# ktzsh/object-tracking

Measured on AMD Instinct MI355X. Metric: frames/sec detect+track @416x416, higher is better.
Workload: dtype f32; 1 GPU; BASELINE.json configs[2]: MultiObjDetTracker (YOLOv2 C=12 + ConvLSTM2D(512) + 1x1 + decode/NMS + track ids), 48 clips x 30 frames per GPU per step, 416x416 uint8; the synthetic head is calibrated to 32 CANDIDATE boxes per frame, of which about 20 survive NMS (config.boxes_per_frame: measured).  The step computes the model's TRACKING output, the one MultiObjDetTracker.predict reads (MultiObjDetTrac; parallelism=clip-shard x1

## Files before the change

object_tracking_amd/build.py:

```python
import os
import subprocess
import sys
from concurrent.futures import ThreadPoolExecutor

HERE = os.path.dirname(os.path.abspath(__file__))
CSRC = os.path.join(HERE, "csrc")
LIB = os.path.join(HERE, "libmi355_dt.so")
HIPCC = os.environ.get("HIPCC", "/opt/rocm/bin/hipcc")

SOURCES = {
    "conv_igemm.hip": [],
    "conv1.hip": [],
    "winograd.hip": [],
    "wino4s_fused.hip": ["-fno-slp-vectorize"],
    "wino_gemm_s3.hip": [],
    "conv3_h2.hip": [],
    "ingest.hip": [],
    "extract.hip": [],
    "exchange.hip": [],
    "decode.hip": ["-ffp-contract=off"],
    "associate.hip": ["-ffp-contract=off"],
    "score.hip": ["-ffp-contract=off"],
    "identity.hip": ["-ffp-contract=off"],
    "detscore.hip": ["-ffp-contract=off"],
    "targets.hip": ["-ffp-contract=off"],
    "recurrent.hip": [],
    "stream_state.hip": [],
    "network.hip": [],
}
COMMON = ["--offload-arch=gfx950", "-O3", "-std=c++17", "-fPIC", "-fvisibility=hidden",
          "-fgpu-rdc" if False else "-fno-gpu-rdc", "-Wall", "-Wno-unused-function"]
HEADERS = [os.path.join(CSRC, "dt_internal.h"), os.path.join(HERE, "..", "include", "mi355_dt.h")]


def _stale(out, deps):
    if not os.path.exists(out):
        return True
    t = os.path.getmtime(out)
    return any(os.path.getmtime(d) > t for d in deps)


def build(force=False, verbose=False):
    objs, jobs = [], []
    for src, extra in SOURCES.items():
        s = os.path.join(CSRC, src)
        o = os.path.join(CSRC, src.replace(".hip", ".o"))
        objs.append(o)
        if force or _stale(o, [s] + HEADERS + [os.path.abspath(__file__)]):
            jobs.append([HIPCC] + COMMON + extra + ["-c", s, "-o", o])

    def run(cmd):
        if verbose:
            print(" ".join(cmd), flush=True)
        r = subprocess.run(cmd, capture_output=True, text=True)
        if r.returncode != 0:
            raise RuntimeError("hipcc failed: %s\n%s\n%s" % (" ".join(cmd), r.stdout, r.stderr))
        if verbose and r.stderr.strip():
            print(r.stderr)

    with ThreadPoolExecutor(max_workers=min(8, max(1, len(jobs)))) as ex:
        list(ex.map(run, jobs))
    if jobs or force or _stale(LIB, objs):
        run([HIPCC, "--offload-arch=gfx950", "-shared", "-fPIC", "-o", LIB] + objs)
    return LIB

# ... 4 lines not shown
```

object_tracking_amd/csrc/conv3_h2.hip:

```cpp
#include "dt_internal.h"
#include <type_traits>

typedef _Float16 c3_h8 __attribute__((ext_vector_type(8)));
typedef _Float16 c3_h4 __attribute__((ext_vector_type(4)));
typedef float c3_f16 __attribute__((ext_vector_type(16)));
typedef float c3_f4 __attribute__((ext_vector_type(4)));
typedef unsigned c3_u4 __attribute__((ext_vector_type(4)));
typedef unsigned c3_u2 __attribute__((ext_vector_type(2)));
typedef __attribute__((address_space(3))) void c3_lptr_t;
typedef const __attribute__((address_space(1))) void c3_gptr_t;

constexpr int C3_PW = 18;
#define C3_THREADS 256
#define C3_NS 3

template <int N>
__device__ __forceinline__ void c3_wait_vm() { __builtin_amdgcn_s_waitcnt(0x0f70 | (N & 15) | ((N >> 4) << 14)); }

__device__ __forceinline__ void c3_mfma(c3_f16 &c, const c3_u4 &w, const c3_u4 &a)
{
    c = __builtin_amdgcn_mfma_f32_32x32x16_f16(__builtin_bit_cast(c3_h8, a), __builtin_bit_cast(c3_h8, w), c, 0, 0, 0);
}

template <int WN, bool POOL, bool FUSE = false>
__global__ __launch_bounds__(C3_THREADS) __attribute__((amdgpu_waves_per_eu(2, 2))) void conv3_h2_kernel(Conv3H2Args p)
{
    static_assert(!FUSE || (WN == 2 && !POOL), "the fused 1x1 follows the 128-channel, un-pooled instance");
    constexpr int WM = 4 / WN;
    constexpr int TH = 4 * WM, TW = 16;
    constexpr int BN = 64 * WN;
    constexpr int PH = TH + 2, PW = C3_PW, NPIX = PH * PW;
    constexpr int PLANE = NPIX * 32;
    constexpr int PATCH = 4 * PLANE;
    constexpr int BPL = BN * 32;
    constexpr int BSTAGE = 4 * BPL;
    constexpr int PB = (4 * BN / 32) / 4;
    constexpr int NJ = (PH * 18 * 8 + C3_THREADS - 1) / C3_THREADS;
    extern __shared__ __attribute__((aligned(16))) unsigned char c3_lds[];
    unsigned char *patch = c3_lds, *bring = c3_lds + PATCH;
    float *btab = reinterpret_cast<float *>(c3_lds + PATCH + C3_NS * BSTAGE);
    [[maybe_unused]] float *btab1 = btab + BN;
    constexpr int SPL = 128 * 32;
    constexpr int BPL1 = 64 * 32;
    const int tid = threadIdx.x, lane = tid & 63, wave = tid >> 6;
    const int wm = wave % WM, wn = wave / WM;
    const int rl = lane & 31, gl = lane >> 5;

    const unsigned am = dt_amax_read(p.amax);
    const float fwd = dt_h2_base(am);
    const float inv = p.pscale[0] * dt_h2_base_inv(am);
    const int nchunk = p.Cin >> 5;
    const int ntn = (p.N + BN - 1) / BN;
    const int tiles = p.tiles_x * p.tiles_y;
    const long long items = (long long)p.B * tiles * ntn;
    const long long wterm = (long long)(9 * p.Cin / 16) * p.Np * 16;
    float out_am = 0.0f;

    long long item = blockIdx.x;
    if (item >= items) return;

    struct Unit { int b, ty0, tx0, n0, chunk; };
    auto unit_of = [&](long long it, int chunk) {
        Unit u;
        u.n0 = (int)(it % ntn) * BN;
        const long long r = it / ntn;
        const int t = (int)(r % tiles);
        u.b = (int)(r / tiles);
        u.ty0 = (t / p.tiles_x) * TH;
        u.tx0 = (t % p.tiles_x) * TW;
        u.chunk = chunk;
        return u;
    };
    c3_f4 pf[NJ];
    auto patch_request = [&](const Unit &u) {
#pragma unroll
        for (int j = 0; j < NJ; ++j) {
// ... 31 lines not shown
    int wdst[PB];
#pragma unroll
    for (int q = 0; q < PB; ++q) {
        const int pc = wave * PB + q;
        const int grp = pc % (BN / 32), ht = pc / (BN / 32);
        const int half = ht >> 1, term = ht & 1;
        wsrc[q] = p.w + term * wterm + ((long long)half * p.Np + 32 * grp + lrow) * 16 + dgran * 8;
        wdst[q] = ht * BPL + grp * 1024;
    }
    const long long wstage = (long long)2 * p.Np * 16;
    auto stage_off = [&](int n0, int chunk, int tap) { return (long long)(chunk * 9 + tap) * wstage + (long long)n0 * 16; };
    auto piece_issue = [&](int buf, long long off, int q) {
        __builtin_amdgcn_global_load_lds((c3_gptr_t *)(wsrc[q] + off), (c3_lptr_t *)(bring + buf * BSTAGE + wdst[q]), 16, 0, 0);
    };
    auto stage_issue = [&](int buf, int n0, int chunk, int tap) {
        const long long off = stage_off(n0, chunk, tap);
#pragma unroll
        for (int q = 0; q < PB; ++q) piece_issue(buf, off, q);
    };
    int offB[2];
#pragma unroll
    for (int j = 0; j < 2; ++j) {
        const int row = wn * 64 + 32 * j + rl;
        offB[j] = (2 * row + (gl ^ ((row >> 3) & 1))) * 16;
    }
    int pixA[2];
#pragma unroll
    for (int i = 0; i < 2; ++i) pixA[i] = (4 * wm + 2 * i + (rl >> 4)) * PW + (rl & 15);
    auto offA_of = [&](int i, int tap) {
        const int pix = pixA[i] + (tap / 3) * PW + tap % 3;
        return pix * 32 + ((gl ^ ((pix >> 3) & 1)) * 16);
    };

    [[maybe_unused]] const unsigned short *w1src[2] = {nullptr, nullptr};
    [[maybe_unused]] int w1dst[2] = {0, 0};
    if constexpr (FUSE) {
        const long long w1term = (long long)8 * p.Np1 * 16;
#pragma unroll
        for (int q = 0; q < 2; ++q) {
            const int pc = wave * 2 + q, grp = pc & 1, ht = pc >> 1, half = ht >> 1, term = ht & 1;
            w1src[q] = p.w1 + term * w1term + ((long long)half * p.Np1 + 32 * grp + lrow) * 16 + dgran * 8;
            w1dst[q] = ht * BPL1 + grp * 1024;
        }
        for (int i = tid; i < 64; i += C3_THREADS) btab1[i] = i < p.N1 ? p.bias1[i] : 0.0f;
    }
    auto fstage_issue = [&](int buf, int q, int k) {
        if constexpr (FUSE)
            __builtin_amdgcn_global_load_lds((c3_gptr_t *)(w1src[k] + (long long)(2 * q) * p.Np1 * 16), (c3_lptr_t *)(bring + buf * BSTAGE + w1dst[k]), 16, 0, 0);
    };
    int sbase = 0;
    auto bufof = [&](int k) { return FUSE ? (sbase + k) % C3_NS : k % C3_NS; };

    Unit cur = unit_of(item, 0);
    patch_request(cur);
    stage_issue(0, cur.n0, 0, 0);
    stage_issue(1, cur.n0, 0, 1);
    for (int i = tid; i < BN; i += C3_THREADS) btab[i] = (cur.n0 + i < p.N) ? p.bias[cur.n0 + i] : 0.0f;
    patch_store();

    c3_f16 acc[2][2];
    c3_u4 fa[2][2][2], fb[2][2][2];
    for (;;) {
        if (cur.chunk == 0) {
#pragma unroll
            for (int j = 0; j < 2; ++j)
#pragma unroll
                for (int i = 0; i < 2; ++i)
#pragma unroll
                    for (int e = 0; e < 16; ++e) acc[j][i][e] = 0.0f;
        }
        const bool last_chunk = cur.chunk == nchunk - 1;
        const long long nitem = last_chunk ? item + gridDim.x : item;
        const bool has_next = nitem < items;
        Unit nxt = cur;
        if (has_next) nxt = unit_of(nitem, last_chunk ? 0 : cur.chunk + 1);

        auto stage = [&](auto tapc) {
            constexpr int tap = decltype(tapc)::value;
            if (tap == 1 && has_next) c3_wait_vm<NJ>();
            else c3_wait_vm<0>();
            __builtin_amdgcn_s_waitcnt(0xc07f);
            __builtin_amdgcn_s_barrier();
            const bool fnext = FUSE && last_chunk && tap >= 7;
            const bool refill = tap < 7 || (has_next && !fnext);
            const long long roff = tap < 7 ? stage_off(cur.n0, cur.chunk, tap + 2) : stage_off(nxt.n0, nxt.chunk, tap - 7);
            const unsigned char *sb = bring + bufof(tap) * BSTAGE, *sn = bring + bufof(tap + 1) * BSTAGE;
            if (tap == 0) {
#pragma unroll
                for (int i = 0; i < 2; ++i)
#pragma unroll
                    for (int t = 0; t < 2; ++t) fa[0][i][t] = *reinterpret_cast<const c3_u4 *>(patch + t * PLANE + offA_of(i, 0));
#pragma unroll
                for (int j = 0; j < 2; ++j)
#pragma unroll
                    for (int t = 0; t < 2; ++t) fb[0][j][t] = *reinterpret_cast<const c3_u4 *>(sb + t * BPL + offB[j]);
            }
            int oa[2], on[2];
#pragma unroll
            for (int i = 0; i < 2; ++i) { oa[i] = offA_of(i, tap); on[i] = offA_of(i, tap < 8 ? tap + 1 : 0); }
            __builtin_amdgcn_sched_barrier(0);
#pragma unroll
            for (int hf = 0; hf < 2; ++hf) {
                const bool rd = hf == 0 || tap < 8;
#pragma unroll
                for (int m = 0; m < 12; ++m) {
                    const int pr = m >> 2, j = (m >> 1) & 1, i = m & 1;
                    c3_mfma(acc[j][i], fb[hf][j][pr == 0 ? 1 : 0], fa[hf][i][pr == 1 ? 1 : 0]);
                    if (rd && m < 8) {
                        const int k = m & 3, blk = k >> 1, t = k & 1;
                        if (m < 4) {
                            if (hf == 0) fa[1][blk][t] = *reinterpret_cast<const c3_u4 *>(patch + (2 + t) * PLANE + oa[blk]);
                            else fa[0][blk][t] = *reinterpret_cast<const c3_u4 *>(patch + t * PLANE + on[blk]);
                        } else {
                            if (hf == 0) fb[1][blk][t] = *reinterpret_cast<const c3_u4 *>(sb + (2 + t) * BPL + offB[blk]);
                            else fb[0][blk][t] = *reinterpret_cast<const c3_u4 *>(sn + t * BPL + offB[blk]);
                        }
                    }
                    if (hf == 0 && m >= 8 && m - 8 < PB && refill) piece_issue(bufof(tap + 2), roff, m - 8);
                    if (FUSE && hf == 0 && m >= 8 && m - 8 < 2 && fnext) fstage_issue(bufof(tap + 2), tap - 7, m - 8);
                    __builtin_amdgcn_sched_barrier(0);
                }
                if (tap == 0 && hf == 0 && has_next) { patch_request(nxt); __builtin_amdgcn_sched_barrier(0); }
            }
        };
        stage(std::integral_constant<int, 0>{}); stage(std::integral_constant<int, 1>{}); stage(std::integral_constant<int, 2>{});
        stage(std::integral_constant<int, 3>{}); stage(std::integral_constant<int, 4>{}); stage(std::integral_constant<int, 5>{});
        stage(std::integral_constant<int, 6>{}); stage(std::integral_constant<int, 7>{}); stage(std::integral_constant<int, 8>{});

        if (FUSE && last_chunk) {
            float am = 0.0f;
#pragma unroll
            for (int j = 0; j < 2; ++j) {
                const float bl = btab[wn * 64 + 32 * j + rl];
#pragma unroll
                for (int i = 0; i < 2; ++i)
#pragma unroll
                    for (int e = 0; e < 16; ++e) {
                        const float z = __builtin_fmaf(acc[j][i][e], inv, bl);
                        const float y = fmaxf(z, z * p.slope);
                        acc[j][i][e] = y;
                        am = fmaxf(am, fabsf(y));
                    }
            }
#pragma unroll
            for (int o = 32; o; o >>= 1) am = fmaxf(am, __shfl_xor(am, o));
            if (lane == 0) btab1[64 + wave] = am;
            __builtin_amdgcn_s_waitcnt(0xc07f);
            __builtin_amdgcn_s_barrier();
            const float tmax = fmaxf(fmaxf(btab1[64], btab1[65]), fmaxf(btab1[66], btab1[67]));
            const unsigned tb = __float_as_uint(tmax);
            const float f1 = dt_h2_base(tb), inv1 = p.pscale1[0] * dt_h2_base_inv(tb);
            c3_f16 acc2[2];
#pragma unroll
            for (int jn = 0; jn < 2; ++jn)
#pragma unroll
                for (int e = 0; e < 16; ++e) acc2[jn][e] = 0.0f;
            const int prow = 32 * wave + rl;
            const int offS = prow * 32 + ((gl ^ ((prow >> 3) & 1)) * 16);
            int offB1[2];
#pragma unroll
            for (int jn = 0; jn < 2; ++jn) { const int n = 32 * jn + rl; offB1[jn] = (2 * n + (gl ^ ((n >> 3) & 1))) * 16; }
#pragma unroll
            for (int q = 0; q < 4; ++q) {
                if (wn == (q >> 1)) {
                    const int j = q & 1, half = rl >> 4, g = (rl >> 3) & 1;
#pragma unroll
                    for (int i = 0; i < 2; ++i)
#pragma unroll
                        for (int r = 0; r < 16; ++r) {
                            const int pp = 64 * wm + 32 * i + 8 * (r >> 2) + 4 * gl + (r & 3);
                            const float x = acc[j][i][r] * f1;
                            const _Float16 hi = (_Float16)x;
                            const _Float16 lo = (_Float16)(x - (float)hi);
                            unsigned char *dst = patch + (half * 2) * SPL + pp * 32 + ((g ^ ((pp >> 3) & 1)) * 16) + (rl & 7) * 2;
                            *reinterpret_cast<_Float16 *>(dst) = hi;
                            *reinterpret_cast<_Float16 *>(dst + SPL) = lo;
                        }
                }
                c3_wait_vm<0>();
                __builtin_amdgcn_s_waitcnt(0xc07f);
                __builtin_amdgcn_s_barrier();
                if (q < 2) { fstage_issue(bufof(11 + q), q + 2, 0); fstage_issue(bufof(11 + q), q + 2, 1); }
                else if (has_next) stage_issue(bufof(11 + q), nxt.n0, nxt.chunk, q - 2);
                const unsigned char *sq = bring + bufof(9 + q) * BSTAGE;
#pragma unroll
                for (int hf = 0; hf < 2; ++hf) {
                    c3_u4 a2[2], b2[2][2];
#pragma unroll
                    for (int t = 0; t < 2; ++t) a2[t] = *reinterpret_cast<const c3_u4 *>(patch + (hf * 2 + t) * SPL + offS);
#pragma unroll
                    for (int jn = 0; jn < 2; ++jn)
#pragma unroll
                        for (int t = 0; t < 2; ++t) b2[jn][t] = *reinterpret_cast<const c3_u4 *>(sq + (hf * 2 + t) * BPL1 + offB1[jn]);
#pragma unroll
                    for (int jn = 0; jn < 2; ++jn) c3_mfma(acc2[jn], b2[jn][1], a2[0]);
#pragma unroll
                    for (int jn = 0; jn < 2; ++jn) c3_mfma(acc2[jn], b2[jn][0], a2[1]);
#pragma unroll
                    for (int jn = 0; jn < 2; ++jn) c3_mfma(acc2[jn], b2[jn][0], a2[0]);
                }
                if (q < 3) {
                    __builtin_amdgcn_s_waitcnt(0xc07f);
                    __builtin_amdgcn_s_barrier();
                }
            }
            sbase = (sbase + 13) % C3_NS;
            const int yb = cur.ty0 + 4 * (wave >> 1) + 2 * (wave & 1);
#pragma unroll
            for (int jn = 0; jn < 2; ++jn) {
                const int n = 32 * jn + rl;
                const float b1 = btab1[n];
                const bool nok = n < p.N1;
#pragma unroll
                for (int r = 0; r < 16; ++r) {
                    const int m = 8 * (r >> 2) + 4 * gl + (r & 3);
                    const int y = yb + (m >> 4), x = cur.tx0 + (m & 15);
                    const float z = __builtin_fmaf(acc2[jn][r], inv1, b1);
                    const float v = fmaxf(z, z * p.slope1);
                    if (nok && y < p.H && x < p.W) {
                        if (p.amax_out) out_am = fmaxf(out_am, fabsf(v));
                        __builtin_nontemporal_store(v, p.out + (long long)cur.b * p.out_bs + ((long long)y * p.W + x) * p.out_ld + n);
                    }
                }
            }
        } else if (last_chunk) {
#pragma unroll
            for (int j = 0; j < 2; ++j) {
                const int nl = wn * 64 + 32 * j + rl;
                const float bl = btab[nl];
                const bool nok = cur.n0 + nl < p.N;
#pragma unroll
                for (int i = 0; i < 2; ++i) {
#pragma unroll
                    for (int e = 0; e < 16; ++e) {
                        const float z = __builtin_fmaf(acc[j][i][e], inv, bl);
                        acc[j][i][e] = fmaxf(z, z * p.slope);
                    }
                    const int yb = cur.ty0 + 4 * wm + 2 * i;
                    if (!POOL) {
#pragma unroll
                        for (int r = 0; r < 16; ++r) {
                            const int m = 8 * (r >> 2) + 4 * gl + (r & 3);
                            const int y = yb + (m >> 4), x = cur.tx0 + (m & 15);
                            if (nok && y < p.H && x < p.W) {
                                if (p.amax_out) out_am = fmaxf(out_am, fabsf(acc[j][i][r]));
                                __builtin_nontemporal_store(acc[j][i][r], p.out + (long long)cur.b * p.out_bs + ((long long)y * p.W + x) * p.out_ld + cur.n0 + nl);
                            }
                        }
                    } else {
                        const int H2 = p.H >> 1, W2 = p.W >> 1;
                        const int y2 = yb >> 1;
#pragma unroll
                        for (int q = 0; q < 4; ++q) {
                            const int r = 2 * q;
                            const float mx = fmaxf(fmaxf(acc[j][i][r], acc[j][i][r + 1]), fmaxf(acc[j][i][r + 8], acc[j][i][r + 9]));
                            const int x2 = (cur.tx0 >> 1) + 4 * (q >> 1) + 2 * gl + (q & 1);
                            if (nok && y2 < H2 && x2 < W2) {
                                if (p.amax_out) out_am = fmaxf(out_am, fabsf(mx));
                                __builtin_nontemporal_store(mx, p.out2 + (((long long)cur.b * H2 + y2) * W2 + x2) * p.out2_ld + cur.n0 + nl);
                            }
                        }
                    }
                }
            }
        }
        if (!has_next) break;
        __builtin_amdgcn_s_waitcnt(0xc07f);
        __builtin_amdgcn_s_barrier();
        patch_store();
        if (last_chunk && nxt.n0 != cur.n0)
            for (int i = tid; i < BN; i += C3_THREADS) btab[i] = (nxt.n0 + i < p.N) ? p.bias[nxt.n0 + i] : 0.0f;
        item = nitem;
        cur = nxt;
    }
    if (p.amax_out) dt_amax_publish(p.amax_out, out_am);
}

bool conv3_h2_usable(const Conv3H2Args &a)
{
    return a.Cin % 32 == 0 && a.Cin >= 32 && a.N >= 64 && a.N % 64 == 0 && a.Np % 64 == 0 && a.in_ld % 4 == 0 && (reinterpret_cast<uintptr_t>(a.in) & 15) == 0 &&
           a.w && a.pscale && a.amax && a.bias && a.zeros && (a.out != nullptr) != (a.out2 != nullptr) && (!a.out2 || !((a.H | a.W) & 1)) &&
           (!a.w1 || (a.N == 128 && a.out && a.pscale1 && a.bias1 && a.N1 > 0 && a.N1 <= 64 && a.Np1 >= 64 && a.Np1 % 32 == 0));
}
double conv3_h2_flops(const Conv3H2Args &a)
{
    const bool wide = a.N % 128 == 0;
    const int th = wide ? 8 : 16;
    const double tiles = (double)a.B * ((a.H + th - 1) / th) * ((a.W + 15) / 16);
    return 6.0 * tiles * th * 16 * (9.0 * a.Cin * a.N + (a.w1 ? (double)a.N * 64 : 0.0));
}

template <int WN, bool POOL, bool FUSE = false>
static int c3_launch(hipStream_t st, const Conv3H2Args &a, int cus)
{
    constexpr int TH = 16 / WN, BN = 64 * WN;
    const size_t lds = (size_t)4 * (TH + 2) * C3_PW * 32 + (size_t)C3_NS * 4 * BN * 32 + BN * 4 + (FUSE ? 68 * 4 : 0);
    static PerDeviceOnce attr;
    if (attr.ensure(nullptr, [&](int) {
            return hipFuncSetAttribute(reinterpret_cast<const void *>(conv3_h2_kernel<WN, POOL, FUSE>), hipFuncAttributeMaxDynamicSharedMemorySize, (int)lds) != hipSuccess;
        }))
        return 1;
    Conv3H2Args p = a;
    p.tiles_y = (a.H + TH - 1) / TH;
// ... 28 lines not shown
```

object_tracking_amd/csrc/dt_internal.h:

```cpp
#pragma once
#include <hip/hip_runtime.h>

#include <atomic>
#include <cstdint>
#include <cstdio>
#include <map>
#include <mutex>
#include <functional>
#include <string>
#include <type_traits>
#include <vector>

#include "../../include/mi355_dt.h"

struct PerDeviceOnce {
    std::atomic<unsigned long long> mask{0};
    std::mutex mu;
    template <class F> int ensure(int *dev_out, F &&setup)
    {
        int dev = -1;
        if (hipGetDevice(&dev) != hipSuccess || dev < 0 || dev > 63) return 1;
        if (dev_out) *dev_out = dev;
        if ((mask.load(std::memory_order_acquire) >> dev) & 1ull) return 0;
        std::lock_guard<std::mutex> lk(mu);
// ... 516 lines not shown
    void reset()
    {
        if (p) (void)hipFree(p);
        p = nullptr;
    }
    hipError_t alloc(size_t n)
    {
        reset();
        const hipError_t e = hipMalloc(reinterpret_cast<void **>(&p), n * sizeof(T));
        if (e != hipSuccess) p = nullptr;
        return e;
    }
    T *get() const { return p; }
    explicit operator bool() const { return p != nullptr; }
};
static_assert(!std::is_copy_constructible<DevMem<float>>::value && !std::is_copy_assignable<DevMem<float>>::value, "a device allocation has one owner");

struct WinoWeights {
    int ts = 0;
    int cin = 0, npad = 0;
    DevMem<float> u;
    DevMem<unsigned short> s3;
    DevMem<unsigned short> h2;
    DevMem<float> h2_pscale;
};

struct ConvLayer {
    int idx = 0, ks = 0, cin = 0, cout = 0, npad = 0;
    DevMem<float> wt;
    DevMem<unsigned short> wt_s3;
    DevMem<unsigned short> bias_s3;
    DevMem<unsigned short> wt_h2;
    DevMem<float> pscale_h2;
    DevMem<unsigned short> w3_h2;
    DevMem<float> pscale_w3;
    WinoWeights wino;
    WinoWeights wino_alt;
    DevMem<float> fused4s;
    DevMem<float> bias;
    DevMem<float> scale;
    bool scale_has_zero = false;
};

struct Policy {
    int wino = 1;
    int wino_tile = 0;
    int wino_mint = 0;
    double wino_ws_gb = 96.0;
    int mosaic = -1;
    int fused4 = 1;
    int trk_merge = 1;
    int pin = 0;
    int c3h2 = 1;
    int conv_cfg = -1;
    int s3_conv1 = 1;
    int s3 = 1;
    int s3_minrows = 2048;
    int s3_minrows_h2 = 64;
    int s3_h2 = 1;
    int c3fuse = 1;
    int h2_minframes = 12;
    int s3_half = 0;
    int s3_rec_minrows = 512;
    int s3_rec_minrows_h2 = 16;
    int s3_1x1_mink = 256;
    int s3_1x1_minrows = 16384;
// ... 98 lines not shown
```

object_tracking_amd/csrc/network.hip:

```cpp
#include <algorithm>
#include <cmath>
#include <cstdarg>
#include <cstdlib>
#include <cstring>
#include <thread>

#include "dt_internal.h"

static const float BN_EPS = 1e-3f;
static const float LEAKY = 0.1f;
static char g_static_err[512] = "";

static const int TRUNK[20][5] = {
    {1, 3, 3, 32, 1},      {2, 3, 32, 64, 1},     {3, 3, 64, 128, 0},    {4, 1, 128, 64, 0},
    {5, 3, 64, 128, 1},    {6, 3, 128, 256, 0},   {7, 1, 256, 128, 0},   {8, 3, 128, 256, 1},
    {9, 3, 256, 512, 0},   {10, 1, 512, 256, 0},  {11, 3, 256, 512, 0},  {12, 1, 512, 256, 0},
    {13, 3, 256, 512, 1},  {14, 3, 512, 1024, 0}, {15, 1, 1024, 512, 0}, {16, 3, 512, 1024, 0},
    {17, 1, 1024, 512, 0}, {18, 3, 512, 1024, 0}, {19, 3, 1024, 1024, 0}, {20, 3, 1024, 1024, 0}};

static inline int round_up(int v, int m) { return (v + m - 1) / m * m; }

int dt_fail(dt_ctx *ctx, int code, const char *fmt, ...)
{
    char buf[512];
    va_list ap;
    va_start(ap, fmt);
    vsnprintf(buf, sizeof(buf), fmt, ap);
    va_end(ap);
    if (ctx) ctx->err = buf;
    else snprintf(g_static_err, sizeof(g_static_err), "%s", buf);
    return code;
}

static void graphs_clear(dt_ctx *ctx)
{
    if (ctx->graphs.empty() && ctx->graph_seen.empty()) return;
    (void)hipStreamSynchronize(ctx->stream);
    for (auto &kv : ctx->graphs) (void)hipGraphExecDestroy(kv.second);
    ctx->graphs.clear();
    ctx->graph_seen.clear();
// ... 500 lines not shown
{
    ConvLayer L;
    L.idx = idx; L.ks = ks; L.cin = cin; L.cout = cout;
    L.npad = round_up(cout, 256);
    std::vector<float> packed((size_t)L.npad * ks * ks * cin);
    pack_conv_weights(hwio, ks, cin, cout, nullptr, cin, nullptr, L.npad, scale, packed.data());
    std::vector<float> bias(L.npad, 0.0f);
    for (int c = 0; c < cout; ++c) bias[c] = bias_src[c];
    int rc = upload(ctx, L.wt, packed);
    if (rc) return rc;
    if (ks == 1 && ctx->pol.s3 != 0 && ctx->pol.s3_1x1 != 0 && cin % 32 == 0 && L.npad % 128 == 0 && cout >= 64) {
        HIP_TRY(ctx, L.wt_s3.alloc(packed.size() * 3));
        if (launch_wino_s3_pack(ctx->stream, L.wt.get(), 1, L.npad, cin, L.wt_s3.get())) return dt_fail(ctx, DT_ERR_DEVICE, "split-bf16 weight pack launch failed");
        HIP_TRY(ctx, hipStreamSynchronize(ctx->stream));
        std::vector<unsigned short> bs((size_t)3 * L.npad * 16, 0);
        for (int n = 0; n < cout; ++n) {
            unsigned short t[3];
            wino_s3_split_host(bias_src[n], t);
            for (int t3 = 0; t3 < 3; ++t3) bs[((size_t)t3 * L.npad + n) * 16] = t[t3];
        }
        if ((rc = upload(ctx, L.bias_s3, bs))) return rc;
        if (!ctx->s3_ones) {
            std::vector<float> ones((size_t)256 * 16, 0.0f);
            for (int r = 0; r < 256; ++r) ones[(size_t)r * 16] = 1.0f;
            if ((rc = upload(ctx, ctx->s3_ones, ones))) return rc;
        }
    }
    if (L.wt_s3 && ctx->pol.s3_h2 != 0) {
        HIP_TRY(ctx, L.wt_h2.alloc(packed.size() * 2));
        HIP_TRY(ctx, L.pscale_h2.alloc(1));
        if (launch_wino_h2_pack(ctx->stream, L.wt.get(), 1, L.npad, cin, 0, amax_slot(ctx, AMAX_PACK), L.wt_h2.get(), L.pscale_h2.get()))
            return dt_fail(ctx, DT_ERR_DEVICE, "fp16-form weight pack launch failed");
        HIP_TRY(ctx, hipStreamSynchronize(ctx->stream));
    }
    if (ks == 3 && (cin == 32 || cin == 64) && cout % 64 == 0 && cout <= 128 && ctx->pol.s3 != 0 && ctx->pol.s3_h2 != 0 && ctx->pol.c3h2 != 0) {
        HIP_TRY(ctx, L.w3_h2.alloc(packed.size() * 2));
        HIP_TRY(ctx, L.pscale_w3.alloc(1));
        if (launch_wino_h2_pack(ctx->stream, L.wt.get(), 1, L.npad, 9 * cin, 0, amax_slot(ctx, AMAX_PACK), L.w3_h2.get(), L.pscale_w3.get()))
            return dt_fail(ctx, DT_ERR_DEVICE, "fp16-form weight pack launch failed");
        HIP_TRY(ctx, hipStreamSynchronize(ctx->stream));
    }
    if (scale) {
        std::vector<float> sc(scale, scale + cout);
        for (float v : sc) L.scale_has_zero |= (v == 0.0f);
        if ((rc = upload(ctx, L.scale, sc))) return rc;
    }
    const bool f4_shape = ((cin == 64 || cin == 128) && cout % 128 == 0 && cout <= 256) || (cin == 32 && cout == 64);
    if (ks == 3 && f4_shape && ctx->pol.wino != 0 && ctx->pol.fused4 != 0) {
        std::vector<float> u36((size_t)36 * L.npad * cin), uf((size_t)36 * cin * cout);
        wino_pack_weights(4, hwio, cin, cout, nullptr, cin, nullptr, L.npad, scale, u36.data());
        wino4s_fused_pack(u36.data(), L.npad, cin, cout, uf.data());
        if ((rc = upload(ctx, L.fused4s, uf))) return rc;
    }
    if (wino_wanted(ctx, ks, cin, cout)) {
        const int ts = wino_tile(ctx, false);
        rc = upload_wino(ctx, L.wino, ts, hwio, cin, cout, nullptr, cin, nullptr, L.npad, scale, ts == 6);
        if (rc) return rc;
        if (ts == 6 && ctx->pol.wino_tile == 0 && cin >= 256) {
            rc = upload_wino(ctx, L.wino_alt, 4, hwio, cin, cout, nullptr, cin, nullptr, L.npad, scale, false);
            if (rc) return rc;
        }
    }
    if ((rc = upload(ctx, L.bias, bias))) return rc;
    (void)hipStreamSynchronize(ctx->stream);
    ctx->layers[idx] = std::move(L);
    return DT_OK;
// ... 406 lines not shown
    return c;
}

struct ConvCall {
    const ConvLayer &L; const float *in; int in_ld, B, H, W; float *out; int out_ld, order, epi; float slope; float *out2; int out2_ld;
    const char *tag; unsigned *amax_out; int M; double flops, bytes;
};

static int conv_s3_1x1(dt_ctx *ctx, const ConvCall &c, bool h2)
{
    const ConvLayer &L = c.L;
    const long long M = (long long)c.B * c.H * c.W;
    GemmS3Args g{};
    g.a_f32 = c.in; g.a_ld = c.in_ld; g.b = L.wt_s3.get(); g.c = c.out; g.c_ps = 0; g.P = 1; g.Mt = (int)M; g.Mp = (int)((M + 255) / 256 * 256); g.N = L.cout; g.Np = L.npad;
    g.half = ctx->pol.s3_half; g.K = L.cin; g.ldc = c.out_ld; g.ones = reinterpret_cast<const unsigned short *>(ctx->s3_ones.get()); g.bias_s3 = L.bias_s3.get(); g.act = 1; g.slope = c.slope;
    if (h2) {
        g.nt = 2; g.b = L.wt_h2.get(); g.pscale = L.pscale_h2.get(); g.bias = L.bias.get(); g.ones = nullptr; g.bias_s3 = nullptr;
        g.amax = ensure_amax(ctx, c.in, M, L.cin, c.in_ld, amax_in_slot(L));
        if (!g.amax) return DT_ERR_DEVICE;
    }
    g.amax_out = c.amax_out;
    prof_count(ctx, h2 ? "s3_form:f16x2" : "s3_form:bf16x3");
    ProfScope ps(ctx, "conv_gemm_s3", wino_gemm_s3_flops(g), 4.0 * M * L.cin + (h2 ? 4.0 : 6.0) * (double)L.cin * L.cout + 4.0 * (double)M * L.cout, c.tag);
    prof_direct_form(ctx, 2.0 * M * (double)L.cin * L.cout, 4.0 * ((double)M * L.cin + (double)L.cin * L.cout + (double)M * L.cout), DF_S3);
    const int rc = launch_wino_gemm_s3(ctx->stream, g, 0);
    return rc ? dt_fail(ctx, launch_code(rc), "%s: split-bf16 1x1 GEMM launch failed (rc=%d)", c.tag, rc) : DT_OK;
}
static int conv_direct_h2(dt_ctx *ctx, const ConvCall &c, const ConvLayer *L4 = nullptr)
{
    const ConvLayer &L = c.L;
    Conv3H2Args a{};
    a.in = c.in; a.in_bs = (long long)c.H * c.W * c.in_ld; a.in_ld = c.in_ld; a.B = c.B; a.H = c.H; a.W = c.W; a.Cin = L.cin; a.N = L.cout; a.Np = L.npad;
    a.w = L.w3_h2.get(); a.pscale = L.pscale_w3.get(); a.bias = L.bias.get(); a.slope = c.slope;
    if (L4) { a.w1 = L4->wt_h2.get(); a.pscale1 = L4->pscale_h2.get(); a.bias1 = L4->bias.get(); a.N1 = L4->cout; a.Np1 = L4->npad; a.slope1 = c.slope; }
    if (c.epi == EPI_POOL) { a.out2 = c.out; a.out2_ld = c.out_ld; }
    else { a.out = c.out; a.out_ld = c.out_ld; a.out_bs = (long long)c.H * c.W * c.out_ld; }
    a.zeros = ws_get(ctx, "zeros256", 256, true);
    if (!a.zeros) return DT_ERR_DEVICE;
    a.amax = ensure_amax(ctx, c.in, (long long)c.B * c.H * c.W, L.cin, c.in_ld, amax_in_slot(L));
    if (!a.amax) return DT_ERR_DEVICE;
    a.amax_out = c.amax_out;
    if (L4) prof_count(ctx, "conv_direct_h2:fused_1x1");
    const double M = c.M;
    ProfScope ps(ctx, "conv_direct_h2", conv3_h2_flops(a),
                 L4 ? 4.0 * (M * L.cin * 1.41 + M * L4->cout)
                    : 4.0 * ((double)c.B * c.H * c.W * L.cin * (L.cout % 128 ? 1.27 : 1.41) * ((L.cout + 127) / 128) + M * L.cout / (c.epi == EPI_POOL ? 4.0 : 1.0)), c.tag);
    if (L4)
        prof_direct_form(ctx, 2.0 * M * (9.0 * L.cin * L.cout + (double)L4->cin * L4->cout),
                         4.0 * (M * L.cin + 9.0 * L.cin * L.cout + 2.0 * M * L.cout + (double)L4->cin * L4->cout + M * L4->cout), DF_C3H2);
    else prof_direct_form(ctx, c.flops, c.bytes, DF_C3H2);
    const int rc = launch_conv3_h2(ctx->stream, a);
    return rc ? dt_fail(ctx, launch_code(rc), L4 ? "%s: fused direct 3x3 + 1x1 launch failed" : "%s: direct fp16-form 3x3 launch failed", c.tag) : DT_OK;
}
static int conv_fused4(dt_ctx *ctx, const ConvCall &c)
{
    const ConvLayer &L = c.L;
    Wino4FusedArgs f{};
    f.in = c.in; f.in_bs = (long long)c.H * c.W * c.in_ld; f.in_ld = c.in_ld; f.B = c.B; f.H = c.H; f.W = c.W; f.Cin = L.cin; f.N = L.cout;
    f.u = L.fused4s.get(); f.bias = L.bias.get(); f.slope = c.slope;
    if (c.epi == EPI_POOL) { f.out2 = c.out; f.out2_ld = c.out_ld; }
    else { f.out = c.out; f.out_ld = c.out_ld; f.out_bs = (long long)c.H * c.W * c.out_ld; }
    const double tiles = (double)c.B * ((c.H + 3) / 4) * ((c.W + 3) / 4);
    ProfScope ps(ctx, "conv_fused", 2.0 * 36.0 * tiles * L.cin * L.cout,
                 4.0 * ((double)c.B * c.H * c.W * L.cin * 1.27 * ((L.cout + 127) / 128) + (double)c.M * L.cout / (c.epi == EPI_POOL ? 4.0 : 1.0)), c.tag);
    prof_direct_form(ctx, c.flops, c.bytes, DF_FUSED);
    float *zeros = ws_get(ctx, "zeros256", 256, true);
    if (!zeros) return DT_ERR_DEVICE;
// ... 55 lines not shown
    int rc = DT_ERR_STATE;
    switch (ch.form) {
    case CF_S3_1X1: rc = conv_s3_1x1(ctx, c, ch.h2); break;
    case CF_DIRECT_H2: rc = conv_direct_h2(ctx, c); break;
    case CF_FUSED4: rc = conv_fused4(ctx, c); break;
    case CF_WINO: rc = conv_wino(ctx, c, *ch.wts, ch.wino); break;
    case CF_SPLITK: case CF_IGEMM: rc = conv_igemm(ctx, c, ch.cfg, ch.ksplit); break;
    }
    if (rc == DT_OK && c.amax_out) amax_note(ctx, lv, amax_out_slot(L));
    return rc;
}

enum { EX_CONV = 0, EX_NORM = 1, EX_ACT = 2, EX_POOL = 3, EX_S2D = 4, EX_CAT = 5 };
struct Extract {
    int idx, kind;
    float *out;
    bool done = false;
};

static int extract_layer(dt_ctx *ctx, const ConvLayer &L, const float *in, int in_ld, int B, int h, int w, Extract &ex)
{
    if (ex.kind == EX_CONV && L.scale && L.scale_has_zero)
        return dt_fail(ctx, DT_ERR_ARG, "conv_%d: a BatchNorm gamma of 0 was folded into the kernel; the raw Conv2D output cannot be recovered", L.idx);
    int rc = run_conv(ctx, L, in, in_ld, B, h, w, ex.out, L.cout, ORD_LINEAR, EPI_PLAIN, ex.kind == EX_ACT ? LEAKY : 1.0f);
    if (rc) return rc;
    if (ex.kind == EX_CONV && L.scale && launch_unfold_bn(ctx->stream, ex.out, (long long)B * h * w, L.cout, L.scale.get(), L.bias.get()))
        return dt_fail(ctx, DT_ERR_DEVICE, "BatchNorm un-fold launch failed");
    ex.done = true;
    return DT_OK;
}

static bool conv34_fusable(const dt_ctx *ctx, const ConvLayer &L3, const ConvLayer &L4, const float *in, int in_ld, int B, int H, int W, const float *out)
{
    return ctx->pol.c3fuse != 0 && L3.ks == 3 && L3.cout == 128 && L4.ks == 1 && L4.cin == 128 && L4.cout <= 64 && L4.wt_h2 && L4.pscale_h2 &&
           choose_conv(ctx, L3, in, in_ld, B, H, W, out, ORD_LINEAR, EPI_PLAIN, false).form == CF_DIRECT_H2;
}
static int run_conv34_fused(dt_ctx *ctx, const ConvLayer &L3, const ConvLayer &L4, const float *in, int in_ld, int B, int H, int W, float *out, int out_ld, float slope)
{
    const Leaves lv = conv_leaves(EPI_PLAIN, out, out_ld, nullptr, 0, (long long)B * H * W, L4.cout);
    amax_forget(ctx, lv);
    char tag[32];
    snprintf(tag, sizeof(tag), "conv_%d", L3.idx);
    const ConvCall c{L3, in, in_ld, B, H, W, out, out_ld, ORD_LINEAR, EPI_PLAIN, slope, nullptr, 0, tag, amax_out_slot(L4) ? amax_slot(ctx, amax_out_slot(L4)) : nullptr, B * H * W, 0.0, 0.0};
    const int rc = conv_direct_h2(ctx, c, &L4);
    if (rc == DT_OK && c.amax_out) amax_note(ctx, lv, amax_out_slot(L4));
    return rc;
}

static int run_trunk(dt_ctx *ctx, int B, float *bufA, float *bufB, float *skip, float *cat, Extract *ex)
{
    const int H = ctx->image_h, W = ctx->image_w;
    float *cur = bufA, *nxt = bufB;
    int h = H / 2, w = W / 2;
    int rc;
    bool cat20 = false;
    for (int li = 1; li < 20; ++li) {
        const int idx = TRUNK[li][0], pool = TRUNK[li][4];
        const ConvLayer &L = ctx->layers[idx];
        if (ex && ex->idx == idx && ex->kind <= EX_ACT) return extract_layer(ctx, L, cur, L.cin, B, h, w, *ex);
        if (idx == 3 && TRUNK[li + 1][0] == 4) {
            const bool ex4 = ex && ex->idx == 4;
            float *out34 = ex4 ? ex->out : nxt;
            if (!(ex4 && ex->kind < EX_ACT) && conv34_fusable(ctx, L, ctx->layers[4], cur, L.cin, B, h, w, out34)) {
                rc = run_conv34_fused(ctx, L, ctx->layers[4], cur, L.cin, B, h, w, out34, ctx->layers[4].cout, LEAKY);
                if (ex4) { ex->done = rc == DT_OK; return rc; }
                if (rc) return rc;
                float *t = cur; cur = nxt; nxt = t;
// ... 1598 lines not shown
```

Before: 17570 frames/s.

## Feed fused 1x1 tail from register accumulators via k-reordered weights

In the fused 3x3+1x1 direct fp16 kernel, the 3x3 MFMA is computed transposed so its accumulators can be split into fp16 hi/lo and fed straight into the 1x1 MFMA as the A operand. This removes the LDS round-trip of the activation tile and the four barrier-separated phases. The 1x1 weights are repacked at load time with a permuted K order so they match the register layout. Each wave group computes partial 1x1 sums over its own half of K, and the halves are exchanged through LDS with a single barrier. The exchange reuses patch and ring-buffer space, which adds layout coupling and a fixed buffer-rotation assumption.

```diff
diff --git a/object_tracking_amd/build.py b/object_tracking_amd/build.py
--- a/object_tracking_amd/build.py
+++ b/object_tracking_amd/build.py
@@ -30,7 +30,7 @@
 }
 COMMON = ["--offload-arch=gfx950", "-O3", "-std=c++17", "-fPIC", "-fvisibility=hidden",
           "-fgpu-rdc" if False else "-fno-gpu-rdc", "-Wall", "-Wno-unused-function"]
-HEADERS = [os.path.join(CSRC, "dt_internal.h"), os.path.join(HERE, "..", "include", "mi355_dt.h")]
+HEADERS = [os.path.join(CSRC, "dt_internal.h"), os.path.join(CSRC, "c3_tail_korder.h"), os.path.join(HERE, "..", "include", "mi355_dt.h")]
 
 
 def _stale(out, deps):
diff --git a/object_tracking_amd/csrc/c3_tail_korder.h b/object_tracking_amd/csrc/c3_tail_korder.h
--- /dev/null
+++ b/object_tracking_amd/csrc/c3_tail_korder.h
@@ -0,0 +1,3 @@
+#pragma once
+
+constexpr int c3_tail_korder(int k) { return (k & ~15) | (((k & 7) >> 2) << 3) | ((k >> 3 & 1) << 2) | (k & 3); }
diff --git a/object_tracking_amd/csrc/conv3_h2.hip b/object_tracking_amd/csrc/conv3_h2.hip
--- a/object_tracking_amd/csrc/conv3_h2.hip
+++ b/object_tracking_amd/csrc/conv3_h2.hip
@@ -5,6 +5,8 @@
 typedef _Float16 c3_h4 __attribute__((ext_vector_type(4)));
 typedef float c3_f16 __attribute__((ext_vector_type(16)));
 typedef float c3_f4 __attribute__((ext_vector_type(4)));
+typedef float c3_f2 __attribute__((ext_vector_type(2)));
+typedef _Float16 c3_h2 __attribute__((ext_vector_type(2)));
 typedef unsigned c3_u4 __attribute__((ext_vector_type(4)));
 typedef unsigned c3_u2 __attribute__((ext_vector_type(2)));
 typedef __attribute__((address_space(3))) void c3_lptr_t;
@@ -20,6 +22,21 @@
 __device__ __forceinline__ void c3_mfma(c3_f16 &c, const c3_u4 &w, const c3_u4 &a)
 {
     c = __builtin_amdgcn_mfma_f32_32x32x16_f16(__builtin_bit_cast(c3_h8, a), __builtin_bit_cast(c3_h8, w), c, 0, 0, 0);
+}
+__device__ __forceinline__ void c3_mfma_t(c3_f16 &c, const c3_u4 &w, const c3_u4 &a)
+{
+    c = __builtin_amdgcn_mfma_f32_32x32x16_f16(__builtin_bit_cast(c3_h8, w), __builtin_bit_cast(c3_h8, a), c, 0, 0, 0);
+}
+__device__ __forceinline__ void c3_split8(const c3_f16 &y, const int e0, const float f, c3_u4 &hi, c3_u4 &lo)
+{
+#pragma unroll
+    for (int q = 0; q < 4; ++q) {
+        const c3_f2 x = c3_f2{y[e0 + 2 * q], y[e0 + 2 * q + 1]} * f;
+        const c3_h2 h = __builtin_convertvector(x, c3_h2);
+        const c3_f2 r = x - __builtin_convertvector(h, c3_f2);
+        hi[q] = __builtin_bit_cast(unsigned, h);
+        lo[q] = __builtin_bit_cast(unsigned, __builtin_convertvector(r, c3_h2));
+    }
 }
 
 template <int WN, bool POOL, bool FUSE = false>
@@ -40,8 +57,9 @@
     unsigned char *patch = c3_lds, *bring = c3_lds + PATCH;
     float *btab = reinterpret_cast<float *>(c3_lds + PATCH + C3_NS * BSTAGE);
     [[maybe_unused]] float *btab1 = btab + BN;
-    constexpr int SPL = 128 * 32;
     constexpr int BPL1 = 64 * 32;
+    constexpr int XPATCH = 16;
+    static_assert(!FUSE || (XPATCH * 1024 <= PATCH && (32 - XPATCH) * 1024 <= BSTAGE), "the exchange: 32 KiB in the patch region and one ring buffer");
     const int tid = threadIdx.x, lane = tid & 63, wave = tid >> 6;
     const int wm = wave % WM, wn = wave / WM;
     const int rl = lane & 31, gl = lane >> 5;
@@ -139,24 +157,19 @@
         return pix * 32 + ((gl ^ ((pix >> 3) & 1)) * 16);
     };
 
-    [[maybe_unused]] const unsigned short *w1src[2] = {nullptr, nullptr};
-    [[maybe_unused]] int w1dst[2] = {0, 0};
+    [[maybe_unused]] const unsigned short *w1lane = nullptr;
     if constexpr (FUSE) {
-        const long long w1term = (long long)8 * p.Np1 * 16;
-#pragma unroll
-        for (int q = 0; q < 2; ++q) {
-            const int pc = wave * 2 + q, grp = pc & 1, ht = pc >> 1, half = ht >> 1, term = ht & 1;
-            w1src[q] = p.w1 + term * w1term + ((long long)half * p.Np1 + 32 * grp + lrow) * 16 + dgran * 8;
-            w1dst[q] = ht * BPL1 + grp * 1024;
-        }
+        w1lane = p.w1 + lrow * 16 + dgran * 8;
         for (int i = tid; i < 64; i += C3_THREADS) btab1[i] = i < p.N1 ? p.bias1[i] : 0.0f;
     }
-    auto fstage_issue = [&](int buf, int q, int k) {
-        if constexpr (FUSE)
-            __builtin_amdgcn_global_load_lds((c3_gptr_t *)(w1src[k] + (long long)(2 * q) * p.Np1 * 16), (c3_lptr_t *)(bring + buf * BSTAGE + w1dst[k]), 16, 0, 0);
-    };
-    int sbase = 0;
-    auto bufof = [&](int k) { return FUSE ? (sbase + k) % C3_NS : k % C3_NS; };
+    auto fpiece_issue = [&](int buf, int h, int q) {
+        if constexpr (FUSE) {
+            const int pc = __builtin_amdgcn_readfirstlane(wave) * 4 + q, grp = pc & 1, kt = pc >> 1, kbl = kt >> 1, term = kt & 1;
+            const long long src = ((long long)(term * 8 + 4 * h + kbl) * p.Np1 + 32 * grp) * 16;
+            __builtin_amdgcn_global_load_lds((c3_gptr_t *)(w1lane + src), (c3_lptr_t *)(bring + buf * BSTAGE + kt * BPL1 + grp * 1024), 16, 0, 0);
+        }
+    };
+    auto bufof = [&](int k) { return k % C3_NS; };
 
     Unit cur = unit_of(item, 0);
     patch_request(cur);
@@ -212,7 +225,8 @@
 #pragma unroll
                 for (int m = 0; m < 12; ++m) {
                     const int pr = m >> 2, j = (m >> 1) & 1, i = m & 1;
-                    c3_mfma(acc[j][i], fb[hf][j][pr == 0 ? 1 : 0], fa[hf][i][pr == 1 ? 1 : 0]);
+                    if constexpr (FUSE) c3_mfma_t(acc[j][i], fb[hf][j][pr == 0 ? 1 : 0], fa[hf][i][pr == 1 ? 1 : 0]);
+                    else c3_mfma(acc[j][i], fb[hf][j][pr == 0 ? 1 : 0], fa[hf][i][pr == 1 ? 1 : 0]);
                     if (rd && m < 8) {
                         const int k = m & 3, blk = k >> 1, t = k & 1;
                         if (m < 4) {
@@ -224,7 +238,7 @@
                         }
                     }
                     if (hf == 0 && m >= 8 && m - 8 < PB && refill) piece_issue(bufof(tap + 2), roff, m - 8);
-                    if (FUSE && hf == 0 && m >= 8 && m - 8 < 2 && fnext) fstage_issue(bufof(tap + 2), tap - 7, m - 8);
+                    if (FUSE && hf == 0 && m >= 8 && fnext) fpiece_issue(bufof(tap + 2), tap - 7, m - 8);
                     __builtin_amdgcn_sched_barrier(0);
                 }
                 if (tap == 0 && hf == 0 && has_next) { patch_request(nxt); __builtin_amdgcn_sched_barrier(0); }
@@ -237,97 +251,100 @@
         if (FUSE && last_chunk) {
             float am = 0.0f;
 #pragma unroll
-            for (int j = 0; j < 2; ++j) {
-                const float bl = btab[wn * 64 + 32 * j + rl];
-#pragma unroll
-                for (int i = 0; i < 2; ++i)
-#pragma unroll
-                    for (int e = 0; e < 16; ++e) {
-                        const float z = __builtin_fmaf(acc[j][i][e], inv, bl);
-                        const float y = fmaxf(z, z * p.slope);
-                        acc[j][i][e] = y;
-                        am = fmaxf(am, fabsf(y));
-                    }
-            }
+            for (int j = 0; j < 2; ++j)
+#pragma unroll
+                for (int c = 0; c < 4; ++c) {
+                    const c3_f4 bl = *reinterpret_cast<const c3_f4 *>(btab + wn * 64 + 32 * j + 8 * c + 4 * gl);
+#pragma unroll
+                    for (int i = 0; i < 2; ++i)
+#pragma unroll
+                        for (int k = 0; k < 4; ++k) {
+                            const float z = __builtin_fmaf(acc[j][i][4 * c + k], inv, bl[k]);
+                            const float y = fmaxf(z, z * p.slope);
+                            acc[j][i][4 * c + k] = y;
+                            am = fmaxf(am, fabsf(y));
+                        }
+                }
 #pragma unroll
             for (int o = 32; o; o >>= 1) am = fmaxf(am, __shfl_xor(am, o));
             if (lane == 0) btab1[64 + wave] = am;
+            c3_wait_vm<0>();
             __builtin_amdgcn_s_waitcnt(0xc07f);
             __builtin_amdgcn_s_barrier();
             const float tmax = fmaxf(fmaxf(btab1[64], btab1[65]), fmaxf(btab1[66], btab1[67]));
             const unsigned tb = __float_as_uint(tmax);
             const float f1 = dt_h2_base(tb), inv1 = p.pscale1[0] * dt_h2_base_inv(tb);
-            c3_f16 acc2[2];
-#pragma unroll
-            for (int jn = 0; jn < 2; ++jn)
-#pragma unroll
-                for (int e = 0; e < 16; ++e) acc2[jn][e] = 0.0f;
-            const int prow = 32 * wave + rl;
-            const int offS = prow * 32 + ((gl ^ ((prow >> 3) & 1)) * 16);
+            c3_f16 acc2[2][2];
             int offB1[2];
 #pragma unroll
-            for (int jn = 0; jn < 2; ++jn) { const int n = 32 * jn + rl; offB1[jn] = (2 * n + (gl ^ ((n >> 3) & 1))) * 16; }
-#pragma unroll
-            for (int q = 0; q < 4; ++q) {
-                if (wn == (q >> 1)) {
-                    const int j = q & 1, half = rl >> 4, g = (rl >> 3) & 1;
-#pragma unroll
-                    for (int i = 0; i < 2; ++i)
-#pragma unroll
-                        for (int r = 0; r < 16; ++r) {
-                            const int pp = 64 * wm + 32 * i + 8 * (r >> 2) + 4 * gl + (r & 3);
-                            const float x = acc[j][i][r] * f1;
-                            const _Float16 hi = (_Float16)x;
-                            const _Float16 lo = (_Float16)(x - (float)hi);
-                            unsigned char *dst = patch + (half * 2) * SPL + pp * 32 + ((g ^ ((pp >> 3) & 1)) * 16) + (rl & 7) * 2;
-                            *reinterpret_cast<_Float16 *>(dst) = hi;
-                            *reinterpret_cast<_Float16 *>(dst + SPL) = lo;
+            for (int s = 0; s < 2; ++s) { const int n = 32 * (wn ^ s) + rl; offB1[s] = (2 * n + (gl ^ ((n >> 3) & 1))) * 16; }
+            const unsigned char *sw = bring + bufof(9 + wn) * BSTAGE;
+            auto xoff = [&](int writer_wn, int i, int c) {
+                const int blk = ((wm * 2 + writer_wn) * 2 + i) * 4 + c;
+                return (blk < XPATCH ? blk * 1024 : PATCH + 2 * BSTAGE + (blk - XPATCH) * 1024) + lane * 16;
+            };
+#pragma unroll
+            for (int it = 0; it < 8; ++it) {
+                const int i = it >> 2, j = (it >> 1) & 1, kb = it & 1;
+                c3_u4 w2[2][2], yh, yl;
+#pragma unroll
+                for (int t = 1; t >= 0; --t)
+#pragma unroll
+                    for (int s = 0; s < 2; ++s) w2[s][t] = *reinterpret_cast<const c3_u4 *>(sw + ((it & 3) * 2 + t) * BPL1 + offB1[s]);
+                c3_split8(acc[j][i], 8 * kb, f1, yh, yl);
+                if ((it & 3) == 0) {
+#pragma unroll
+                    for (int s = 0; s < 2; ++s)
+#pragma unroll
+                        for (int e = 0; e < 16; ++e) acc2[s][i][e] = 0.0f;
+                }
+#pragma unroll
+                for (int s = 0; s < 2; ++s) c3_mfma(acc2[s][i], yh, w2[s][1]);
+#pragma unroll
+                for (int s = 0; s < 2; ++s) c3_mfma(acc2[s][i], yl, w2[s][0]);
+#pragma unroll
+                for (int s = 0; s < 2; ++s) c3_mfma(acc2[s][i], yh, w2[s][0]);
+                if ((it & 3) == 3) {
+#pragma unroll
+                    for (int c = 0; c < 4; ++c)
+                        *reinterpret_cast<c3_f4 *>(c3_lds + xoff(wn, i, c)) = c3_f4{acc2[1][i][4 * c], acc2[1][i][4 * c + 1], acc2[1][i][4 * c + 2], acc2[1][i][4 * c + 3]};
+                }
+                __builtin_amdgcn_sched_barrier(0);
+            }
+            __builtin_amdgcn_s_waitcnt(0xc07f);
+            __builtin_amdgcn_s_barrier();
+            const bool v4 = !((p.out_ld | p.out_bs | p.N1) & 3) && !(reinterpret_cast<uintptr_t>(p.out) & 15);
+#pragma unroll
+            for (int i = 0; i < 2; ++i) {
+                const int y = cur.ty0 + 4 * wm + 2 * i + (rl >> 4), x = cur.tx0 + (rl & 15);
+                const bool pok = y < p.H && x < p.W;
+                float *dst = p.out + (long long)cur.b * p.out_bs + ((long long)y * p.W + x) * p.out_ld;
+#pragma unroll
+                for (int c = 0; c < 4; ++c) {
+                    const int n = 32 * wn + 8 * c + 4 * gl;
+                    const c3_f4 o = *reinterpret_cast<const c3_f4 *>(c3_lds + xoff(wn ^ 1, i, c));
+                    const c3_f4 b1 = *reinterpret_cast<const c3_f4 *>(btab1 + n);
+                    c3_f4 v;
+#pragma unroll
+                    for (int k = 0; k < 4; ++k) {
+                        const float z = __builtin_fmaf(acc2[0][i][4 * c + k] + o[k], inv1, b1[k]);
+                        v[k] = fmaxf(z, z * p.slope1);
+                    }
+                    if (v4) {
+                        if (pok && n < p.N1) {
+                            if (p.amax_out) out_am = fmaxf(out_am, fmaxf(fmaxf(fabsf(v[0]), fabsf(v[1])), fmaxf(fabsf(v[2]), fabsf(v[3]))));
+                            __builtin_nontemporal_store(v, reinterpret_cast<c3_f4 *>(dst + n));
                         }
-                }
-                c3_wait_vm<0>();
-                __builtin_amdgcn_s_waitcnt(0xc07f);
-                __builtin_amdgcn_s_barrier();
-                if (q < 2) { fstage_issue(bufof(11 + q), q + 2, 0); fstage_issue(bufof(11 + q), q + 2, 1); }
-                else if (has_next) stage_issue(bufof(11 + q), nxt.n0, nxt.chunk, q - 2);
-                const unsigned char *sq = bring + bufof(9 + q) * BSTAGE;
-#pragma unroll
-                for (int hf = 0; hf < 2; ++hf) {
-                    c3_u4 a2[2], b2[2][2];
-#pragma unroll
-                    for (int t = 0; t < 2; ++t) a2[t] = *reinterpret_cast<const c3_u4 *>(patch + (hf * 2 + t) * SPL + offS);
-#pragma unroll
-                    for (int jn = 0; jn < 2; ++jn)
-#pragma unroll
-                        for (int t = 0; t < 2; ++t) b2[jn][t] = *reinterpret_cast<const c3_u4 *>(sq + (hf * 2 + t) * BPL1 + offB1[jn]);
-#pragma unroll
-                    for (int jn = 0; jn < 2; ++jn) c3_mfma(acc2[jn], b2[jn][1], a2[0]);
-#pragma unroll
-                    for (int jn = 0; jn < 2; ++jn) c3_mfma(acc2[jn], b2[jn][0], a2[1]);
-#pragma unroll
-                    for (int jn = 0; jn < 2; ++jn) c3_mfma(acc2[jn], b2[jn][0], a2[0]);
-                }
-                if (q < 3) {
-                    __builtin_amdgcn_s_waitcnt(0xc07f);
-                    __builtin_amdgcn_s_barrier();
-                }
-            }
-            sbase = (sbase + 13) % C3_NS;
-            const int yb = cur.ty0 + 4 * (wave >> 1) + 2 * (wave & 1);
-#pragma unroll
-            for (int jn = 0; jn < 2; ++jn) {
-                const int n = 32 * jn + rl;
-                const float b1 = btab1[n];
-                const bool nok = n < p.N1;
-#pragma unroll
-                for (int r = 0; r < 16; ++r) {
-                    const int m = 8 * (r >> 2) + 4 * gl + (r & 3);
-                    const int y = yb + (m >> 4), x = cur.tx0 + (m & 15);
-                    const float z = __builtin_fmaf(acc2[jn][r], inv1, b1);
-                    const float v = fmaxf(z, z * p.slope1);
-                    if (nok && y < p.H && x < p.W) {
-                        if (p.amax_out) out_am = fmaxf(out_am, fabsf(v));
-                        __builtin_nontemporal_store(v, p.out + (long long)cur.b * p.out_bs + ((long long)y * p.W + x) * p.out_ld + n);
+                    } else {
+#pragma unroll
+                        for (int k = 0; k < 4; ++k)
+                            if (pok && n + k < p.N1) {
+                                if (p.amax_out) out_am = fmaxf(out_am, fabsf(v[k]));
+                                __builtin_nontemporal_store(v[k], dst + n + k);
+                            }
                     }
+                    if (has_next) piece_issue(bufof((i * 4 + c) >> 2), stage_off(nxt.n0, nxt.chunk, (i * 4 + c) >> 2), (i * 4 + c) & 3);
+                    __builtin_amdgcn_sched_barrier(0);
                 }
             }
         } else if (last_chunk) {
@@ -375,7 +392,7 @@
         __builtin_amdgcn_s_waitcnt(0xc07f);
         __builtin_amdgcn_s_barrier();
         patch_store();
-        if (last_chunk && nxt.n0 != cur.n0)
+        if (!FUSE && last_chunk && nxt.n0 != cur.n0)
             for (int i = tid; i < BN; i += C3_THREADS) btab[i] = (nxt.n0 + i < p.N) ? p.bias[nxt.n0 + i] : 0.0f;
         item = nitem;
         cur = nxt;
diff --git a/object_tracking_amd/csrc/dt_internal.h b/object_tracking_amd/csrc/dt_internal.h
--- a/object_tracking_amd/csrc/dt_internal.h
+++ b/object_tracking_amd/csrc/dt_internal.h
@@ -572,6 +572,7 @@
     DevMem<unsigned short> bias_s3;
     DevMem<unsigned short> wt_h2;
     DevMem<float> pscale_h2;
+    DevMem<unsigned short> wt_h2k;
     DevMem<unsigned short> w3_h2;
     DevMem<float> pscale_w3;
     WinoWeights wino;
diff --git a/object_tracking_amd/csrc/network.hip b/object_tracking_amd/csrc/network.hip
--- a/object_tracking_amd/csrc/network.hip
+++ b/object_tracking_amd/csrc/network.hip
@@ -6,6 +6,7 @@
 #include <thread>
 
 #include "dt_internal.h"
+#include "c3_tail_korder.h"
 
 static const float BN_EPS = 1e-3f;
 static const float LEAKY = 0.1f;
@@ -572,6 +573,17 @@
         if (launch_wino_h2_pack(ctx->stream, L.wt.get(), 1, L.npad, cin, 0, amax_slot(ctx, AMAX_PACK), L.wt_h2.get(), L.pscale_h2.get()))
             return dt_fail(ctx, DT_ERR_DEVICE, "fp16-form weight pack launch failed");
         HIP_TRY(ctx, hipStreamSynchronize(ctx->stream));
+        if (cin == 128 && cout <= 64) {
+            std::vector<float> korder(packed.size());
+            for (int n = 0; n < L.npad; ++n)
+                for (int k = 0; k < cin; ++k) korder[(size_t)n * cin + k] = packed[(size_t)n * cin + c3_tail_korder(k)];
+            DevMem<float> wk;
+            if ((rc = upload(ctx, wk, korder))) return rc;
+            HIP_TRY(ctx, L.wt_h2k.alloc(packed.size() * 2));
+            if (launch_wino_h2_pack(ctx->stream, wk.get(), 1, L.npad, cin, 0, amax_slot(ctx, AMAX_PACK), L.wt_h2k.get(), nullptr))
+                return dt_fail(ctx, DT_ERR_DEVICE, "fp16-form weight pack launch failed");
+            HIP_TRY(ctx, hipStreamSynchronize(ctx->stream));
+        }
     }
     if (ks == 3 && (cin == 32 || cin == 64) && cout % 64 == 0 && cout <= 128 && ctx->pol.s3 != 0 && ctx->pol.s3_h2 != 0 && ctx->pol.c3h2 != 0) {
         HIP_TRY(ctx, L.w3_h2.alloc(packed.size() * 2));
@@ -1044,7 +1056,7 @@
     Conv3H2Args a{};
     a.in = c.in; a.in_bs = (long long)c.H * c.W * c.in_ld; a.in_ld = c.in_ld; a.B = c.B; a.H = c.H; a.W = c.W; a.Cin = L.cin; a.N = L.cout; a.Np = L.npad;
     a.w = L.w3_h2.get(); a.pscale = L.pscale_w3.get(); a.bias = L.bias.get(); a.slope = c.slope;
-    if (L4) { a.w1 = L4->wt_h2.get(); a.pscale1 = L4->pscale_h2.get(); a.bias1 = L4->bias.get(); a.N1 = L4->cout; a.Np1 = L4->npad; a.slope1 = c.slope; }
+    if (L4) { a.w1 = L4->wt_h2k.get(); a.pscale1 = L4->pscale_h2.get(); a.bias1 = L4->bias.get(); a.N1 = L4->cout; a.Np1 = L4->npad; a.slope1 = c.slope; }
     if (c.epi == EPI_POOL) { a.out2 = c.out; a.out2_ld = c.out_ld; }
     else { a.out = c.out; a.out_ld = c.out_ld; a.out_bs = (long long)c.H * c.W * c.out_ld; }
     a.zeros = ws_get(ctx, "zeros256", 256, true);
@@ -1166,7 +1178,7 @@
 
 static bool conv34_fusable(const dt_ctx *ctx, const ConvLayer &L3, const ConvLayer &L4, const float *in, int in_ld, int B, int H, int W, const float *out)
 {
-    return ctx->pol.c3fuse != 0 && L3.ks == 3 && L3.cout == 128 && L4.ks == 1 && L4.cin == 128 && L4.cout <= 64 && L4.wt_h2 && L4.pscale_h2 &&
+    return ctx->pol.c3fuse != 0 && L3.ks == 3 && L3.cout == 128 && L4.ks == 1 && L4.cin == 128 && L4.cout <= 64 && L4.wt_h2k && L4.pscale_h2 &&
            choose_conv(ctx, L3, in, in_ld, B, H, W, out, ORD_LINEAR, EPI_PLAIN, false).form == CF_DIRECT_H2;
 }
 static int run_conv34_fused(dt_ctx *ctx, const ConvLayer &L3, const ConvLayer &L4, const float *in, int in_ld, int B, int H, int W, float *out, int out_ld, float slope)
```

Result: no change. 17540 frames/s (-0.2%).
